# yaomy533/pose_estimation

Measured on AMD Instinct MI355X. Metric: crops/sec at 640×480 RGB-D, 1000 sampled pts; ADD(-S) AUC vs reference, higher is better.
Workload: dtype f32; 1 GPU; LineMOD 'cat' batch=64/GPU, 120x120 crops from 640x480 RGB-D, HRNet-W18 + 1000-pt fusion + TBase, PnP-RANSAC (H=100) on GPU; batch_per_gpu=64, global_batch=64, crop=120, points=1000, backbone=hrnet_w18, parallelism=single, graph=True, micro_batches=1, pipeline=none, graph_branches=True

## Files before the change

pose_estimation_amd/csrc/winograd4.hip:

```cpp
#include "krrn_common.h"
#include "krrn_split.h"

namespace {

constexpr int kGX = 16, kGY = 2, kT = kGX * kGY;
constexpr int kN = 64;
constexpr int kC = 8;
constexpr int kRR = 4 * kGY + 2, kRC = 4 * kGX + 2;
constexpr int kRS = 152;
constexpr int kRing = 1536;
constexpr int kRingF = kRing * 4;
constexpr int kVMH = 36 * 64 * 4;
constexpr int kVL = 36 * 64 * 2;
constexpr int kET = kN * 4;
constexpr unsigned kOOB = 0xFFFF0000u;
constexpr int kRawK = 6;
constexpr int kGap = 6;
static_assert(kRR * kRS <= kRing && kRing == 3 * 512, "raw ring");
static_assert(2 * (kRC - 1) + 1 + (kRC - 1) / 4 < kRS && (kRS * 4) % 16 == 0, "padded raw row");
constexpr int kOffL = 2 * kVMH * 4;
constexpr int kOffR = kOffL + 2 * kVL * 4;
constexpr int kLdsBytes = kOffR + 2 * kRingF * 4;
static_assert(36 * 16 * kET <= kLdsBytes, "epilogue (16 tiles) fits the LDS");

struct Wino4Args {
  const float* in;
  int in_cs, in_co;
  int B, H, W, cin;
  long long img;
  const void* U3;
  int N, n_store;
  const float* scale;
  const float* bias;
  const float* res;
  int res_cs, res_co;
  float* out;
  int out_cs, out_co;
  int relu;
  int vec;
  int Ht, Wt;
  const float* w1;
  float* part;
};

template <int CTRL>
__device__ __forceinline__ float dpp_f(float x) {
  return __int_as_float(__builtin_amdgcn_update_dpp(0, __float_as_int(x), CTRL, 0xF, 0xF, false));
}

__device__ __forceinline__ u32x6 split3(const f32x4 x) {
  const KrrnSplit3 s = krrn_split3(x);
  return u32x6{s.m0, s.m1, s.h0, s.h1, s.l0, s.l1};
}

template <int K, typename V>
__device__ __forceinline__ V bt_row(const V (&x)[6]) {
// ... 1 lines not shown
#pragma unroll
  for (int e = 0; e < (int)(sizeof(V) / 4); ++e) {
    if constexpr (K == 0) y[e] = __builtin_fmaf(4.f, x[0][e], __builtin_fmaf(-5.f, x[2][e], x[4][e]));
    if constexpr (K == 1) y[e] = __builtin_fmaf(-4.f, x[1][e] + x[2][e], x[3][e] + x[4][e]);
    if constexpr (K == 2) y[e] = __builtin_fmaf(4.f, x[1][e] - x[2][e], x[4][e] - x[3][e]);
    if constexpr (K == 3) y[e] = __builtin_fmaf(2.f, x[3][e] - x[1][e], x[4][e] - x[2][e]);
    if constexpr (K == 4) y[e] = __builtin_fmaf(2.f, x[1][e] - x[3][e], x[4][e] - x[2][e]);
    if constexpr (K == 5) y[e] = __builtin_fmaf(4.f, x[1][e], __builtin_fmaf(-5.f, x[3][e], x[5][e]));
  }
  return y;
}
template <int K>
__device__ __forceinline__ constexpr bool bt_uses(int c) {
  return K == 0 ? (c == 0 || c == 2 || c == 4) : (K == 5 ? (c == 1 || c == 3 || c == 5) : (c >= 1 && c <= 4));
}

template <int I>
__device__ __forceinline__ f32x4 at_row(const f32x4 (&x)[6]) {
  f32x4 y;
#pragma unroll
  for (int e = 0; e < 4; ++e) {
    if constexpr (I == 0) y[e] = ((x[0][e] + x[1][e]) + x[2][e]) + (x[3][e] + x[4][e]);
    if constexpr (I == 1) y[e] = __builtin_fmaf(2.f, x[3][e] - x[4][e], x[1][e] - x[2][e]);
    if constexpr (I == 2) y[e] = __builtin_fmaf(4.f, x[3][e] + x[4][e], x[1][e] + x[2][e]);
    if constexpr (I == 3) y[e] = __builtin_fmaf(8.f, x[3][e] - x[4][e], x[1][e] - x[2][e]) + x[5][e];
  }
  return y;
}
template <int I>
__device__ __forceinline__ constexpr bool at_uses(int u) {
  return I == 0 ? (u <= 4) : (I == 3 ? (u >= 1) : (u >= 1 && u <= 4));
}

template <int I, int HP>
__device__ __forceinline__ void epi_row(const Wino4Args& a, const char* E, int nq, int tl, int pass, int b, int ty0,
                                        int tx0, int ng, int nb) {
  const char* eb = E + tl * kET + nq * 16;
  f32x4 t[6];
#pragma unroll
  for (int v = 0; v < 6; ++v) {
    f32x4 m[6];
#pragma unroll
    for (int u = 0; u < 6; ++u)
      m[u] = at_uses<I>(u) ? *reinterpret_cast<const f32x4*>(eb + (6 * u + v) * 16 * kET) : f32x4{0.f, 0.f, 0.f, 0.f};
    t[v] = at_row<I>(m);
    asm volatile("" : "+v"(t[v])::"memory");
  }
  f32x4 y[4];
  y[0] = at_row<0>(t);
  y[1] = at_row<1>(t);
  y[2] = at_row<2>(t);
  y[3] = at_row<3>(t);
  const int tile = 16 * pass + tl;
  const int ty = ty0 + (tile >> 4), tx = tx0 + (tile & 15);
  const int oy = 4 * ty + I;
  const int nj = min(4, a.W - 4 * tx);
  if constexpr (HP > 0) {
    const bool ok = ty < a.Ht && oy < a.H && nj > 0 && ng < a.n_store;
    const f32x4 zero = {0.f, 0.f, 0.f, 0.f};
    const f32x4 scl = ok && a.scale ? *reinterpret_cast<const f32x4*>(a.scale + ng) : f32x4{1.f, 1.f, 1.f, 1.f};
    const f32x4 bia = ok && a.bias ? *reinterpret_cast<const f32x4*>(a.bias + ng) : zero;
    f32x4 w[HP];
#pragma unroll
    for (int o = 0; o < HP; ++o) w[o] = ok ? *reinterpret_cast<const f32x4*>(a.w1 + (size_t)o * a.N + ng) : zero;
    const long long pix = ((long long)b * a.H + oy) * a.W + 4 * tx;
    float s[4][HP];
#pragma unroll
    for (int j = 0; j < 4; ++j) {
      const bool okj = ok && j < nj;
      f32x4 v;
#pragma unroll
      for (int e = 0; e < 4; ++e) v[e] = __builtin_fmaf(y[j][e], scl[e], bia[e]);
      if (a.res && okj) v += *reinterpret_cast<const f32x4*>(a.res + (pix + j) * a.res_cs + a.res_co + ng);
      if (a.relu) {
#pragma unroll
        for (int e = 0; e < 4; ++e) v[e] = fmaxf(v[e], 0.f);
      }
      if (!okj) v = zero;
#pragma unroll
      for (int o = 0; o < HP; ++o) s[j][o] = v[0] * w[o][0] + v[1] * w[o][1] + v[2] * w[o][2] + v[3] * w[o][3];
    }
    const bool b0 = nq & 1, b1 = (nq >> 1) & 1;
    float t1[2][HP];
#pragma unroll
    for (int jj = 0; jj < 2; ++jj)
#pragma unroll
      for (int o = 0; o < HP; ++o) {
// ... 37 lines not shown
      }
      *reinterpret_cast<f32x4*>(o + j * a.out_cs) = v;
    }
    return;
  }
#pragma unroll
  for (int e = 0; e < 4; ++e) {
    if (ng + e >= a.n_store) break;
    const float scl = a.scale ? a.scale[ng + e] : 1.f, bia = a.bias ? a.bias[ng + e] : 0.f;
#pragma unroll
    for (int j = 0; j < 4; ++j) {
      if (j >= nj) break;
      float v = __builtin_fmaf(y[j][e], scl, bia);
      if (rs) v += rs[j * a.res_cs + e];
      if (a.relu) v = fmaxf(v, 0.f);
      o[j * a.out_cs + e] = v;
    }
  }
}

__global__ __launch_bounds__(256) void wino4_head_finish_kernel(const float* __restrict__ part, int nbn, long long M,
                                                                int HW, const float* __restrict__ b1, int p1,
                                                                float* __restrict__ out, int out_c) {
  const long long m = (long long)blockIdx.x * 256 + threadIdx.x;
  if (m >= M) return;
  f32x4 v = *reinterpret_cast<const f32x4*>(part + m * 4);
  for (int nb = 1; nb < nbn; ++nb) v += *reinterpret_cast<const f32x4*>(part + ((size_t)nb * M + m) * 4);
  const long long b = m / HW, p = m - b * HW;
#pragma unroll
  for (int o = 0; o < 4; ++o)
    if (o < p1) out[(b * out_c + o) * HW + p] = v[o] + (b1 ? b1[o] : 0.f);
}

template <int HP>
__global__ __launch_bounds__(512, 1) void wino_f43_x3_kernel(const Wino4Args a) {
  __shared__ __attribute__((aligned(16))) char smem[kLdsBytes];
  const int tid = threadIdx.x, lane = tid & 63;
  const int wave = __builtin_amdgcn_readfirstlane(tid >> 6);
  const int gxn = krrn_cdiv(a.Wt, kGX), gyn = krrn_cdiv(a.Ht, kGY), nbn = krrn_cdiv(a.N, kN);
  const int per_img = gxn * gyn;
  const int bid = krrn_xcd_remap(blockIdx.x, a.B * per_img * nbn);
  const int sp = bid / nbn, nb = bid - (bid / nbn) * nbn;
  const int b = sp / per_img, r2 = sp - (sp / per_img) * per_img;
  const int by = r2 / gxn, bx = r2 - (r2 / gxn) * gxn;
  const int n0 = nb * kN;
  const int ty0 = by * kGY, tx0 = bx * kGX;
  const int nck = a.cin / kC;

  const __amdgpu_buffer_rsrc_t rsA = __builtin_amdgcn_make_buffer_rsrc(
      (void*)(a.in + (size_t)b * a.img + a.in_co), (short)0, (int)min(a.img * 4 - (long long)a.in_co * 4, 0x7FFFFFFFLL),
      0x00020000);
  unsigned roff[3];
#pragma unroll
  for (int i = 0; i < 3; ++i) {
    const int s = 192 * wave + 64 * i + lane;
    const int r = s / kRS, q = s - (s / kRS) * kRS;
    const int g4 = q / 9, w9 = q - (q / 9) * 9;
    const int col = 4 * g4 + (w9 >> 1), hh = w9 & 1;
    const int iy = 4 * ty0 - 1 + r, ix = 4 * tx0 - 1 + col;
    const bool ok = r < kRR && w9 < 8 && col < kRC && iy >= 0 && iy < a.H && ix >= 0 && ix < a.W;
    roff[i] = ok ? (unsigned)((((long long)iy * a.W + ix) * a.in_cs + 4 * hh) * 4) : kOOB;
  }
  auto dma_raw = [&](int ck, int slot) {
    char* dst = smem + kOffR + slot * (kRingF * 4) + 3 * 1024 * wave;
#pragma unroll
    for (int i = 0; i < 3; ++i)
      __builtin_amdgcn_raw_ptr_buffer_load_lds(rsA, (__attribute__((address_space(3))) void*)(dst + 1024 * i), 16,
                                               roff[i], ck * kC * 4, 0, 0);
  };

  const int g = wave & 3, nh = wave >> 2;
  const int cu0 = 3 * (g >> 1), cv0 = 3 * (g & 1);
  const int fr = lane & 31, h = lane >> 5;
  const long long nrec = (long long)nck * 36 * a.N * 2;
  const char* u3 = reinterpret_cast<const char*>(a.U3);
  const __amdgpu_buffer_rsrc_t rsMH =
      __builtin_amdgcn_make_buffer_rsrc((void*)u3, (short)0, (int)min(nrec * 16, 0x7FFFFFFFLL), 0x00020000);
  const __amdgpu_buffer_rsrc_t rsL =
      __builtin_amdgcn_make_buffer_rsrc((void*)(u3 + nrec * 16), (short)0, (int)min(nrec * 8, 0x7FFFFFFFLL), 0x00020000);
  const unsigned wrec = (unsigned)(2 * min(n0 + 32 * nh + fr, a.N - 1) + h);
  u32x4 wmh[3];
  u32x2 wl[3];
  auto load_w = [&](int ck, int k) {
    ck = min(ck, nck - 1);
    const int comp = 6 * (cu0 + k / 3) + cv0 + k % 3;
    const unsigned srec = (unsigned)((ck * 36 + comp) * a.N * 2);
    wmh[k % 3] = __builtin_bit_cast(u32x4, __builtin_amdgcn_raw_buffer_load_b128(rsMH, wrec * 16u, srec * 16u, 0));
    wl[k % 3] = __builtin_bit_cast(u32x2, __builtin_amdgcn_raw_buffer_load_b64(rsL, wrec * 8u, srec * 8u, 0));
  };

  f32x16 acc[9];
#pragma unroll
  for (int k = 0; k < 9; ++k)
#pragma unroll
    for (int r = 0; r < 16; ++r) acc[k][r] = 0.f;

  const int tv = wave < 6 ? wave : 5;
  int tcol[4];
  float tk[4];
  switch (tv) {
    case 0: tcol[0] = 0; tcol[1] = 2; tcol[2] = 4; tcol[3] = 4; tk[0] = 4.f; tk[1] = -5.f; tk[2] = 1.f; tk[3] = 0.f; break;
    case 1: tcol[0] = 1; tcol[1] = 2; tcol[2] = 3; tcol[3] = 4; tk[0] = -4.f; tk[1] = -4.f; tk[2] = 1.f; tk[3] = 1.f; break;
    case 2: tcol[0] = 1; tcol[1] = 2; tcol[2] = 3; tcol[3] = 4; tk[0] = 4.f; tk[1] = -4.f; tk[2] = -1.f; tk[3] = 1.f; break;
    case 3: tcol[0] = 1; tcol[1] = 2; tcol[2] = 3; tcol[3] = 4; tk[0] = -2.f; tk[1] = -1.f; tk[2] = 2.f; tk[3] = 1.f; break;
    case 4: tcol[0] = 1; tcol[1] = 2; tcol[2] = 3; tcol[3] = 4; tk[0] = 2.f; tk[1] = -1.f; tk[2] = -2.f; tk[3] = 1.f; break;
    default: tcol[0] = 1; tcol[1] = 3; tcol[2] = 5; tcol[3] = 5; tk[0] = 4.f; tk[1] = -5.f; tk[2] = 1.f; tk[3] = 0.f; break;
  }
  const int ttile = lane & 31, th = lane >> 5;
  const int pbase = (4 * (ttile >> 4)) * kRS + 9 * (ttile & 15) + th;
  const char* tb[4];
  char* twm = nullptr;
  char* twl = nullptr;
  f32x4 td[4];
  f32x4 te[6];
  auto t_begin = [&](int ck) {
    const int p = ck & 1;
    const char* rb = smem + kOffR + p * (kRingF * 4) + 16 * pbase;
#pragma unroll
    for (int t = 0; t < 4; ++t) tb[t] = rb + 16 * (2 * tcol[t] + (tcol[t] >> 2));
    twm = smem + p * (kVMH * 4) + tv * 1024 + 16 * lane;
    twl = smem + kOffL + p * (kVL * 4) + tv * 512 + 8 * lane;
#pragma unroll
    for (int t = 0; t < 4; ++t) td[t] = *reinterpret_cast<const f32x4*>(tb[t]);
  };
  auto t_step = [&](int s) {
    if (s < 6) {
#pragma unroll
      for (int e = 0; e < 4; ++e)
        te[s][e] = __builtin_fmaf(tk[3], td[3][e], __builtin_fmaf(tk[2], td[2][e], __builtin_fmaf(tk[1], td[1][e], tk[0] * td[0][e])));
      if (s < 5) {
#pragma unroll
        for (int t = 0; t < 4; ++t) {
          (void)tv;
          td[t] = *reinterpret_cast<const f32x4*>(tb[t] + (s + 1) * kRS * 16);
        }
      }
      return;
    }
    const int u = s - 6;
    f32x4 x;
    switch (u) {
      case 0: x = bt_row<0>(te); break;
      case 1: x = bt_row<1>(te); break;
      case 2: x = bt_row<2>(te); break;
      case 3: x = bt_row<3>(te); break;
      case 4: x = bt_row<4>(te); break;
      default: x = bt_row<5>(te); break;
    }
    const u32x6 ch = split3(x);
    *reinterpret_cast<u32x4*>(twm + 6 * u * 1024) = u32x4{ch[0], ch[1], ch[2], ch[3]};
    *reinterpret_cast<u32x2*>(twl + 6 * u * 512) = u32x2{ch[4], ch[5]};
  };
  constexpr int kStep0[10] = {0, 1, 2, 3, 4, 5, 7, 9, 11, 12};

  auto comp_of = [&](int k) { return 6 * (cu0 + k / 3) + cv0 + k % 3; };
  auto do_chunk = [&](int ck) {
    const bool tr = ck + 1 < nck && wave < 6;
    const int p = ck & 1;
    const char* vm = smem + p * (kVMH * 4) + 16 * lane;
    const char* vlo = smem + kOffL + p * (kVL * 4) + 8 * lane;
    auto chain = [&](int k) {
      const u32x4 mh = *reinterpret_cast<const u32x4*>(vm + comp_of(k) * 1024);
      const u32x2 l = *reinterpret_cast<const u32x2*>(vlo + comp_of(k) * 512);
      return u32x6{mh[0], mh[1], mh[2], mh[3], l[0], l[1]};
    };
    const bool stage = ck + 2 < nck;
    __builtin_amdgcn_sched_barrier(0);
    if (tr) t_begin(ck + 1 < nck ? ck + 1 : ck + 1 - 2);
    u32x6 acn = chain(0);
#pragma unroll
    for (int k = 0; k < 9; ++k) {
      u32x6 ac = acn;
      if (k < 8) acn = chain(k + 1);
      asm volatile("" : "+v"(ac));
      u32x6 bc = {wmh[k % 3][0], wmh[k % 3][1], wmh[k % 3][2], wmh[k % 3][3], wl[k % 3][0], wl[k % 3][1]};
      asm volatile("" : "+v"(bc));
      acc[k] = __builtin_amdgcn_mfma_f32_32x32x16_bf16(krrn_sub4(ac, 0), krrn_sub4(bc, 0), acc[k], 0, 0, 0);
      acc[k] = __builtin_amdgcn_mfma_f32_32x32x16_bf16(krrn_sub4(ac, 0), krrn_sub4(bc, 2), acc[k], 0, 0, 0);
      acc[k] = __builtin_amdgcn_mfma_f32_32x32x16_bf16(krrn_sub4(ac, 2), krrn_sub4(bc, 0), acc[k], 0, 0, 0);
      if (k < 6) load_w(ck, k + 3); else load_w(ck + 1, k - 6);
      if (tr) {
#pragma unroll
        for (int st = kStep0[k]; st < kStep0[k + 1]; ++st) t_step(st);
      }
      if (k == kRawK && stage) dma_raw(ck + 2, p);
      __builtin_amdgcn_sched_group_barrier(0x100, 6, 0);
      __builtin_amdgcn_sched_group_barrier(0x008, 1, 0);
      __builtin_amdgcn_sched_group_barrier(0x002, kGap, 0);
      __builtin_amdgcn_sched_group_barrier(0x008, 1, 0);
      __builtin_amdgcn_sched_group_barrier(0x002, kGap, 0);
      __builtin_amdgcn_sched_group_barrier(0x008, 1, 0);
      __builtin_amdgcn_sched_group_barrier(0x002, kGap, 0);
      __builtin_amdgcn_sched_barrier(0);
    }
  };

  dma_raw(0, 0);
  if (nck > 1) dma_raw(1, 1);
#pragma unroll
  for (int k = 0; k < 3; ++k) load_w(0, k);
  if (nck > 1)
    asm volatile("s_waitcnt vmcnt(9)\n\ts_barrier" ::: "memory");
  else
    asm volatile("s_waitcnt vmcnt(6)\n\ts_barrier" ::: "memory");
  if (wave < 6) {
    t_begin(0);
#pragma unroll
    for (int st = 0; st < 12; ++st) t_step(st);
  }
  asm volatile("s_waitcnt vmcnt(6) lgkmcnt(0)\n\ts_barrier" ::: "memory");

  for (int ck = 0; ck < nck; ++ck) {
    do_chunk(ck);
    static_assert(kRawK >= 6 && kRawK <= 8, "vmcnt count below");
    asm volatile("s_waitcnt vmcnt(%0) lgkmcnt(0)\n\ts_barrier" ::"n"(2 * (8 - kRawK)) : "memory");
  }

  const int enq = lane & 15, etl = lane >> 4, ei = wave & 3;
#pragma unroll
  for (int pass = 0; pass < 2; ++pass) {
    char* ew = smem + (32 * nh + fr) * 4;
#pragma unroll
    for (int k = 0; k < 9; ++k) {
      const int comp = comp_of(k);
#pragma unroll
      for (int q = 0; q < 8; ++q) {
        const int r = 8 * pass + q;
        const int tl = (r & 3) + 8 * ((r >> 2) & 1) + 4 * h;
        *reinterpret_cast<float*>(ew + (comp * 16 + tl) * kET) = acc[k][r];
      }
    }
    __syncthreads();
#pragma unroll
    for (int it = 0; it < 2; ++it) {
      const int tl = 4 * ((wave >> 2) + 2 * it) + etl;
      const int ng = n0 + 4 * enq;
      switch (ei) {
        case 0: epi_row<0, HP>(a, smem, enq, tl, pass, b, ty0, tx0, ng, nb); break;
        case 1: epi_row<1, HP>(a, smem, enq, tl, pass, b, ty0, tx0, ng, nb); break;
        case 2: epi_row<2, HP>(a, smem, enq, tl, pass, b, ty0, tx0, ng, nb); break;
        default: epi_row<3, HP>(a, smem, enq, tl, pass, b, ty0, tx0, ng, nb); break;
      }
    }
    __syncthreads();
  }
}

}

KRRN_API int krrn_conv3x3_wino4_x3_f32(const float* in, int in_cs, int in_co, int B, int H, int W, int cin,
                                       const void* U3, int N, int n_store, const float* scale, const float* bias,
                                       const float* res, int res_cs, int res_co, float* out, int out_cs, int out_co,
                                       int relu, void* stream) {
  if (!in || !U3 || !out) return KRRN_EARG;
  if (B < 1 || H < 1 || W < 1 || N < 1 || n_store < 1 || n_store > N) return KRRN_ESHAPE;
  if (cin < kC || (cin % kC) || in_co + cin > in_cs) return KRRN_EALIGN;
  if (!krrn_aligned16(U3) || (((uintptr_t)in) & 15u) || (in_cs & 3) || (in_co & 3)) return KRRN_EALIGN;
  if (out_co + n_store > out_cs) return KRRN_ESHAPE;
  Wino4Args a;
  a.in = in; a.in_cs = in_cs; a.in_co = in_co; a.B = B; a.H = H; a.W = W; a.cin = cin;
  a.img = (long long)H * W * in_cs;
  a.U3 = U3; a.N = N; a.n_store = n_store; a.scale = scale; a.bias = bias;
  a.res = res; a.res_cs = res_cs; a.res_co = res_co;
  a.out = out; a.out_cs = out_cs; a.out_co = out_co; a.relu = relu;
  a.Ht = (H + 3) / 4; a.Wt = (W + 3) / 4;
  const bool ov = !(out_cs & 3) && !(out_co & 3) && krrn_aligned16(out);
  const bool rv = !res || (!(res_cs & 3) && !(res_co & 3) && krrn_aligned16(res));
  const bool sv = (!scale || krrn_aligned16(scale)) && (!bias || krrn_aligned16(bias));
  a.vec = (ov && rv && sv) ? 1 : 0;
  a.w1 = nullptr; a.part = nullptr;
  const long long nrec = (long long)(cin / kC) * 36 * N * 2;
  if (a.img * 4 >= 0x7FFF0000LL || nrec * 16 >= 0x7FFF0000LL) return KRRN_ESHAPE;
  const long long rb = (long long)B * krrn_cdiv(a.Ht, kGY) * krrn_cdiv(a.Wt, kGX) * krrn_cdiv(N, kN);
  if (rb > 0x7fffffffLL) return KRRN_ESHAPE;
  hipLaunchKernelGGL(wino_f43_x3_kernel<0>, dim3((unsigned)rb), dim3(512), 0, (hipStream_t)stream, a);
  return krrn_launch_status();
}

KRRN_API int krrn_conv3x3_wino4_x3_head_f32(const float* in, int in_cs, int in_co, int B, int H, int W, int cin,
                                            const void* U3, int N, const float* scale, const float* bias,
                                            const float* res, int res_cs, int res_co, int relu, const float* w1,
                                            const float* b1, int p1, float* part, float* out, int out_c,
                                            void* stream) {
  if (!in || !U3 || !w1 || !part || !out) return KRRN_EARG;
  if (B < 1 || H < 1 || W < 1 || N < 4 || (N & 3) || p1 < 1 || p1 > 4 || out_c < p1) return KRRN_ESHAPE;
  if (cin < kC || (cin % kC) || in_co + cin > in_cs) return KRRN_EALIGN;
  if (!krrn_aligned16(U3) || (((uintptr_t)in) & 15u) || (in_cs & 3) || (in_co & 3)) return KRRN_EALIGN;
  if (!krrn_aligned16(w1) || !krrn_aligned16(part)) return KRRN_EALIGN;
  if ((scale && !krrn_aligned16(scale)) || (bias && !krrn_aligned16(bias))) return KRRN_EALIGN;
  if (res && ((res_cs & 3) || (res_co & 3) || !krrn_aligned16(res))) return KRRN_EALIGN;
  Wino4Args a;
  a.in = in; a.in_cs = in_cs; a.in_co = in_co; a.B = B; a.H = H; a.W = W; a.cin = cin;
  a.img = (long long)H * W * in_cs;
  a.U3 = U3; a.N = N; a.n_store = N; a.scale = scale; a.bias = bias;
  a.res = res; a.res_cs = res_cs; a.res_co = res_co;
  a.out = nullptr; a.out_cs = 0; a.out_co = 0; a.relu = relu; a.vec = 1;
  a.Ht = (H + 3) / 4; a.Wt = (W + 3) / 4;
  a.w1 = w1; a.part = part;
  const long long nrec = (long long)(cin / kC) * 36 * N * 2;
  if (a.img * 4 >= 0x7FFF0000LL || nrec * 16 >= 0x7FFF0000LL) return KRRN_ESHAPE;
  const int nbn = krrn_cdiv(N, kN);
  const long long rb = (long long)B * krrn_cdiv(a.Ht, kGY) * krrn_cdiv(a.Wt, kGX) * nbn;
  const long long M = (long long)B * H * W;
  const long long fb = (M + 255) / 256;
  if (rb > 0x7fffffffLL || fb > 0x7fffffffLL) return KRRN_ESHAPE;
  hipStream_t s = (hipStream_t)stream;
  if (p1 <= 3) hipLaunchKernelGGL(wino_f43_x3_kernel<3>, dim3((unsigned)rb), dim3(512), 0, s, a);
  else hipLaunchKernelGGL(wino_f43_x3_kernel<4>, dim3((unsigned)rb), dim3(512), 0, s, a);
  const int st = krrn_launch_status();
  if (st != KRRN_OK) return st;
  hipLaunchKernelGGL(wino4_head_finish_kernel, dim3((unsigned)fb), dim3(256), 0, s, part, nbn, M, H * W, b1, p1, out,
                     out_c);
  return krrn_launch_status();
}
```

pose_estimation_amd/hrnet.py:

```python
from __future__ import annotations

from typing import List, Optional, Tuple

import torch
import torch.nn as nn

from . import knobs, ops
from .config import load_hrnet_spec
from .ops import Act, pad4
from .runtime import add_conv_group, add_gemm, Plan, add_conv, ptr

FUSE_EDGES = knobs.flag("KRRN_FUSE_EDGES")
FUSE_EARLY = knobs.flag("KRRN_FUSE_EARLY")
MODULE_STREAMS = knobs.flag("KRRN_MODULE_STREAMS")
STAGE_STREAMS = knobs.flag("KRRN_STAGE_STREAMS")
CONVT_KCHUNK = 16

BN_MOMENTUM = 0.1


def conv3x3(cin, cout, stride=1):
    return nn.Conv2d(cin, cout, kernel_size=3, stride=stride, padding=1, bias=False)


# ... 121 lines not shown
                if cur[i] != pre[i]:
                    layers.append(nn.Sequential(nn.Conv2d(pre[i], cur[i], 3, 1, 1, bias=False),
                                                nn.BatchNorm2d(cur[i]), nn.ReLU(True)))
                else:
                    layers.append(None)
            else:
                chain = []
                for j in range(i + 1 - len(pre)):
                    cin = pre[-1]
                    cout = cur[i] if j == i - len(pre) else cin
                    chain.append(nn.Sequential(nn.Conv2d(cin, cout, 3, 2, 1, bias=False), nn.BatchNorm2d(cout),
                                               nn.ReLU(True)))
                layers.append(nn.Sequential(*chain))
        return nn.ModuleList(layers)


def build_hrnet(cfg) -> HRNet:
    return HRNet(load_hrnet_spec(cfg.Module.BACKBONE), cfg.Module.BACKBONE_OUTC)



class _Builder:
    def __init__(self, plan: Plan, B: int):
        self.plan = plan
        self.B = B
        self.dev = plan.device
        self.specs = []

    def act(self, H, W, c, cs=None) -> Act:
        cs = pad4(c) if cs is None else cs
        t = self.plan.buf((self.B, H, W, cs))
        return Act(t, self.B, H, W, cs, 0, c)

    def conv(self, x: Act, conv: nn.Module, bn: Optional[nn.Module], out: Optional[Act] = None,
             res: Optional[Act] = None, relu: bool = False, cin_map=None) -> Act:
        if isinstance(conv, nn.ConvTranspose2d):
            spec = ops.make_convT(conv, bn, self.dev, cin_map=cin_map, cin_p=x.cp)
        else:
            spec = ops.make_conv(conv, bn, self.dev, cin_map=cin_map, cin_p=x.cp)
        self.specs.append(spec)
        Ho, Wo = ops.conv_out_hw(spec, x.H, x.W)
        if out is None:
            out = self.act(Ho, Wo, spec.cout)
        assert (out.H, out.W) == (Ho, Wo) and out.cp >= pad4(spec.cout)
        wino = ops.wino_eligible(spec, x.B * Ho * Wo)
        if wino and ops.wino4_eligible(spec, x, Ho, Wo):
            self.emit_wino(x, conv, spec, out, res, relu, f4=True, cin_map=cin_map)
        elif wino and x.cs % 2 == 0 and x.co % 2 == 0:
            self.emit_wino(x, conv, spec, out, res, relu, f4=False, cin_map=cin_map)
        elif ops.small_conv_eligible(spec, x):
            self.emit_small(x, spec, out, res, relu)
        elif not self.emit_gemm(x, spec, out, res, relu):
            self.emit_conv(x, spec, out, res, relu)
        return out

    def wino_problem(self, x: Act, conv: nn.Conv2d, spec, f4: bool, cin_map=None) -> Tuple[torch.Tensor, dict]:
        t, comps = (4, 36) if f4 else (2, 16)
        np_ = pad4(spec.cout)
        U = ops.wino_weights_x3((ops.wino4_weights if f4 else ops.wino_weights)(conv, self.dev, cin_map=cin_map,
                                                                                cin_p=x.cp))
        self.specs.append(U)
        pipe = 2.0 * comps * spec.cin_p * np_ * x.B * ((x.H + t - 1) // t) * ((x.W + t - 1) // t)
        return U, dict(kernel="wino_f43_x3" if f4 else "wino_f23_x3", M=x.B * x.H * x.W, N=np_, K=spec.cin_p * 9,
                       mfma_flops=pipe * 6 / 16, mfma_bf16_flops=pipe * 6)

    def conv_head(self, x: Act, conv: nn.Module, bn: Optional[nn.Module], final: nn.Conv2d, out: torch.Tensor,
                  n_store: int) -> bool:
        if not (isinstance(conv, nn.Conv2d) and tuple(final.kernel_size) == (1, 1)
                and tuple(final.stride) == (1, 1) and final.in_channels == conv.out_channels
                and n_store <= min(4, final.out_channels) and x.cs % 2 == 0 and x.co % 2 == 0):
            return False
        spec = ops.make_conv(conv, bn, self.dev, cin_p=x.cp)
        M = x.B * x.H * x.W
        if not ops.wino_eligible(spec, M):
            return False
        np_ = pad4(spec.cout)
        f4 = ops.wino4_eligible(spec, x, x.H, x.W)
        U, meta = self.wino_problem(x, conv, spec, f4)
        w1 = torch.zeros(4, np_, device=self.dev)
        w1[:final.out_channels, :spec.cout] = final.weight.detach().reshape(final.out_channels, -1).float().to(self.dev)
        b1 = None
        if final.bias is not None:
            b1 = torch.zeros(4, device=self.dev)
            b1[:final.out_channels] = final.bias.detach().float().to(self.dev)
        self.specs += [spec, w1] + ([b1] if b1 is not None else [])
        part = self.plan.scratch(((np_ + 63) // 64) * M * 4)
        meta.update(kernel=meta["kernel"] + "_head", tag="conv_wino_head",
                    flops=2.0 * spec.cin * spec.cout * 9 * M + 2.0 * spec.cout * n_store * M)
        self.plan.add("krrn_conv3x3_wino4_x3_head_f32" if f4 else "krrn_conv3x3_wino_x3_head_f32", ptr(x.t), x.cs,
                      x.co, x.B, x.H, x.W, spec.cin_p, ptr(U), np_,
                      ptr(spec.scale), ptr(spec.bias), ptr(None), 0, 0, 1, ptr(w1), ptr(b1), n_store, ptr(part),
                      ptr(out), out.shape[1], meta=meta)
        return True

    def upsample2(self, x: Act) -> Act:
        up = self.act(2 * x.H, 2 * x.W, x.c)
        self.resize(x, up, align=True)
        return up

    def emit_gemm(self, x: Act, spec, out: Act, res: Optional[Act], relu: bool) -> bool:
        if not (spec.kind == "conv" and spec.ksize == 1 and spec.stride == 1 and out.co == 0
                and (res is None or res.co == 0)):
            return False
        np_ = pad4(spec.cout)
        return add_gemm(self.plan, a=x.t, a_off=x.co, lda=x.cs, M=x.B * x.H * x.W, wt=spec.wt[0], K=spec.cin_p,
                        N=np_, scale=spec.scale, bias=spec.bias, out=out.t, ldo=out.cs, relu=relu,
                        res=res.t if res is not None else None, ldr=res.cs if res is not None else 0,
                        cin=spec.cin, cout=spec.cout, tag="conv1x1_gemm")

    @staticmethod
    def small_problem(x: Act, spec, out: Act, res: Optional[Act], relu: bool) -> dict:
        np_ = pad4(spec.cout)
        M = x.B * out.H * out.W
        taps = spec.ksize * spec.ksize
        ntiles = (np_ + 15) // 16
        nw, ks = ops.small_conv_config(M, ntiles, spec.cin_p)
        ksteps = (taps * spec.cin_p // 4 + 3) // 4
        return dict(x=ptr(x.t), in_cs=x.cs, in_co=x.co, B=x.B, H=x.H, W=x.W, cin=spec.cin_p, wt=ptr(spec.wt[0]),
                    N=np_, n_store=np_, scale=ptr(spec.scale), bias=ptr(spec.bias),
                    res=ptr(res.t) if res is not None else ptr(None), res_cs=res.cs if res is not None else 0,
                    res_co=res.co if res is not None else 0, out=ptr(out.t), out_cs=out.cs, out_co=out.co,
                    relu=int(relu), ksize=spec.ksize, stride=spec.stride, nw=nw, ks=ks, M=M,
                    flops=2.0 * spec.cin * spec.cout * taps * M,
                    mfma_flops=2.0 * 16 * ksteps * ops.small_conv_rows(np_, ksteps, ks) * M)

    def emit_small(self, x: Act, spec, out: Act, res: Optional[Act], relu: bool, tag: str = "conv"):
        p = self.small_problem(x, spec, out, res, relu)
        self.plan.add("krrn_conv_small_f32", p["x"], p["in_cs"], p["in_co"], p["B"], p["H"], p["W"], p["cin"], p["wt"],
                      p["N"], p["n_store"], p["scale"], p["bias"], p["res"], p["res_cs"], p["res_co"], p["out"],
                      p["out_cs"], p["out_co"], p["relu"], p["ksize"], p["stride"], p["nw"], p["ks"],
                      meta=dict(kernel=f"conv_small<{p['nw']},{p['ks']}>", flops=p["flops"], tag=tag, M=p["M"], N=p["N"],
                                K=spec.cin_p * spec.ksize ** 2, splits=1, mfma_flops=p["mfma_flops"]))

    def emit_wino(self, x: Act, conv: nn.Conv2d, spec, out: Act, res: Optional[Act], relu: bool, f4: bool,
                  cin_map=None):
        U, meta = self.wino_problem(x, conv, spec, f4, cin_map)
        np_ = meta["N"]
        meta.update(flops=2.0 * spec.cin * spec.cout * 9 * meta["M"], tag="conv_wino")
        self.plan.add("krrn_conv3x3_wino4_x3_f32" if f4 else "krrn_conv3x3_wino_x3_f32", ptr(x.t), x.cs, x.co, x.B,
                      x.H, x.W, spec.cin_p, ptr(U), np_, np_, ptr(spec.scale), ptr(spec.bias),
                      ptr(res.t) if res is not None else ptr(None), res.cs if res is not None else 0,
                      res.co if res is not None else 0, ptr(out.t), out.cs, out.co, int(relu), meta=meta)

    def emit_convT_s2(self, x: Act, spec, out: Act, relu: bool, tag: str = "conv"):
        U3, table = ops.convT_weights_x3(spec)
        self.specs.append(U3)
        taps = sum(len(t) for t in spec.taps)
        grid = x.B * (-(-x.H // 4) * 4) * (-(-x.W // 32) * 32)
        issued = 2.0 * grid * 128 * spec.cin_p * max(len(t) for t in spec.taps) * 4
        meta = dict(kernel="convt_s2_x3", flops=2.0 * spec.cin * spec.cout * taps * x.B * x.H * x.W,
                    tag=tag + "_convT", M=x.B * x.H * x.W * 4, N=128, K=spec.cin_p * taps,
                    mfma_flops=issued * 6 / 16, mfma_bf16_flops=issued * 6)
        self.plan.add("krrn_convT_s2_x3_f32", ptr(x.t), x.cs, x.co, x.B, x.H, x.W, spec.cin_p, table, ptr(U3), 128,
                      ptr(spec.scale), ptr(spec.bias), int(relu), ptr(out.t), out.cs, out.co, out.H, out.W, meta=meta)

    def emit_conv(self, x: Act, spec, out: Act, res: Optional[Act], relu: bool, tag: str = "conv"):
        np_ = pad4(spec.cout)
        if ops.convT_s2_eligible(spec, x, out, res):
            self.emit_convT_s2(x, spec, out, relu, tag)
            return
        if spec.kind == "convT" and 1 < len(spec.taps) <= 4:
            probs = [dict(x=ptr(x.t), x_cs=x.cs, x_co=x.co, B=x.B, Hi=x.H, Wi=x.W, cin_p=spec.cin_p, Hg=x.H, Wg=x.W,
                          in_s=1, taps=taps, wt=ptr(spec.wt[cls]), N=np_, n_store=np_, scale=ptr(spec.scale),
                          bias=ptr(spec.bias), res=ptr(res.t) if res is not None else None,
                          res_cs=res.cs if res is not None else 0, res_co=res.co if res is not None else 0,
                          out=ptr(out.t), out_cs=out.cs, out_co=out.co, Ho=out.H, Wo=out.W, osy=2, osx=2, ooy=ooy,
                          oox=oox, relu=relu, cin=spec.cin, cout=spec.cout)
                     for cls, (taps, (ooy, oox)) in enumerate(zip(spec.taps, spec.cls_off))]
            q = CONVT_KCHUNK if CONVT_KCHUNK and spec.cin_p % CONVT_KCHUNK == 0 else 0
            wts = [ops.kchunk_weights(w, len(t), spec.cin_p, q) for w, t in zip(spec.wt, spec.taps)] if q else spec.wt
            for pr in probs:
                pr["k_chunk"] = q
            for pr, cls in zip(probs, range(len(probs))):
                w3 = ops.conv_weights_x3(wts[cls])
                self.specs.append(w3)
# ... 211 lines not shown
```

pose_estimation_amd/krrn.py:

```python
from __future__ import annotations

import ctypes
from collections import OrderedDict

from typing import Dict, List, Optional, Sequence, Tuple

import torch
import torch.nn as nn

from . import knobs, ops
from .config import CONFIG
from .fusion import FEAT_SID, FusionNetLite, build_fusion_plan, emit_fusion_cloud_part, level_sizes
from .hrnet import _Builder, build_hrnet, build_hrnet_plan
from .ops import Act, pad4
from .posenet import PoseNet, build_tbase_plan, emit_pair_compact, emit_tbase_level1
from .runtime import Late, Plan, RngStream, add_conv, h2d, ptr



TBASE_EARLY = knobs.flag("KRRN_TBASE_EARLY")
GRAPH = knobs.flag("KRRN_GRAPH")
FUSION_EARLY = knobs.flag("KRRN_FUSION_EARLY")


# ... 108 lines not shown
                    tb_pre.update(emit_tbase_level1(model.pose.t_net, plan, B, N, N1, fb["feat1"], fb["feat2"],
                                                      cls_key="cls", inc_r=cfg.Module.POSENet.INC_R, num_cls=C))

            if TBASE_EARLY:
                hooks["level1"].append(tracked(emit_tb_l1))
            tb_pairs = {}
            hooks["pairs"] = [tracked(lambda fb: tb_pairs.update(
                emit_pair_compact(plan, B, N, N1, N2, fb["nn1"], fb["nn2"]) or {}))]
            f0 = len(plan.ops)
            feat, self.fusion_bufs = build_fusion_plan(model.fusion, plan, B, N, self.p9, self.perms, hooks=hooks,
                                                       materialize=model.keep_fusion_feat, early=early)
            self.fusion_op_ids = {id(op) for op in plan.ops[f0:] if id(op) not in side_ids and op.name != "sync"}
            self.fusion_op_ids |= early_ids
            self.feat = feat
            fb = self.fusion_bufs
            levels = dict(fm5=fb["fm5"], feat1=fb["feat1"], feat2=fb["feat2"], nn1=fb["nn1"], nn2=fb["nn2"], N1=N1,
                          N2=N2)
            self.pred_t, self.tbase_bufs = build_tbase_plan(model.pose.t_net, plan, B, N, "cls", "cloud",
                                                            cfg.Module.POSENet.INC_R, C, levels,
                                                            pre=tb_pre or None, pre_sid=tb_sid,
                                                            pairs=tb_pairs or None)
            if feat is not None:
                plan.join([FEAT_SID])
        if pose_hook is not None:
            plan.join([psid])
        self.env = {"cls": self.cls, "cloud": self.cloud}
        self.graph: Optional[torch.cuda.CUDAGraph] = None
        self.warm = False
        self.nbytes = plan_bytes(plan) + plan_bytes(getattr(self, "device_perm_plan", None))

    def _head_tail(self, bld: _Builder, x: Act, convs, final: nn.Conv2d, out: torch.Tensor, n_store: int):
        spec = ops.make_conv(final, None, self.plan.device, cin_p=pad4(convs[-1][0].out_channels))
        bld.specs.append(spec)
        h = bld.upsample2(x)
        for i, (conv, bn) in enumerate(convs):
            if i == len(convs) - 1 and bld.conv_head(h, conv, bn, final, out, n_store):
                return
            h = bld.conv(h, conv, bn, relu=True)
        self._nchw_conv(h, spec, out, n_store)

    def _nchw_conv(self, x: Act, spec, out: torch.Tensor, n_store: int):
        B, Cx, Ho, Wo = out.shape
        np_ = pad4(spec.cout)
        if len(spec.taps[0]) == 1 and spec.stride == 1 and spec.cin_p <= 256 and np_ <= 80:
            name, wt = "krrn_conv1x1_nchw_f32", spec.wt[0]
            if spec.cin_p == 128 and np_ > 48:
                name, wt = "krrn_conv1x1_nchw_x3_f32", ops.quad_weights_x3(spec.wt[0], np_, 128)
                self.plan.buffers.append(wt)
            self.plan.add(name, ptr(x.t), x.cs, x.co, x.B, Ho * Wo, spec.cin_p, ptr(wt), np_,
                          n_store, ptr(spec.scale), ptr(spec.bias), ptr(out), Cx, 0,
                          meta=dict(kernel="conv1x1_nchw", flops=2.0 * spec.cin * n_store * B * Ho * Wo,
                                    tag="head_final", M=B * Ho * Wo, N=np_, K=spec.cin_p, splits=1,
                                    mfma_flops=2.0 * spec.cin_p * 16 * ((np_ + 15) // 16) * B * Ho * Wo))
            return
        add_conv(self.plan, x=ptr(x.t), x_cs=x.cs, x_co=x.co, B=x.B, Hi=x.H, Wi=x.W, cin_p=spec.cin_p, Hg=Ho, Wg=Wo,
                 in_s=spec.stride, taps=spec.taps[0], wt=ptr(spec.wt[0]), N=pad4(spec.cout), n_store=n_store,
                 scale=ptr(spec.scale), bias=ptr(spec.bias), out=ptr(out), out_cs=Cx, out_co=0, Ho=Ho, Wo=Wo,
                 nchw=True, cin=spec.cin, cout=n_store, tag="head_final")

    def load_inputs(self, x, p_emb, choose, cls):
        self.x_in.copy_(x, non_blocking=True)
        if self.opt_pose:
            self.cloud.copy_(p_emb, non_blocking=True)
            self.choose.copy_(choose.reshape(self.B, 1, self.N), non_blocking=True)
        self.cls.copy_(cls.reshape(self.B, 1), non_blocking=True)

    def set_perms(self, perms: Optional[Sequence[torch.Tensor]], mode: str):
        if not self.opt_pose:
            return
        if perms is not None:
            for (k, n, m), p in zip(self.perm_sizes, perms):
# ... 171 lines not shown
```

Baseline: 6766 crops/s.

## Fuse 2x bilinear upsample into Winograd F(4,3) conv input transform for head

Adds an UP variant of the Winograd F(4,3) kernel that reads the half-resolution input directly and folds the bilinear upsample weights into the input transform coefficients. This removes the separate upsample2 kernel and its full-resolution intermediate buffer in the head tail. The tile shape changes to 32x1 with a smaller source window per block, and the transform stage uses precomputed per-tile combined coefficients. In exchange it adds coefficient setup cost and a different LDS window layout, and it relies on the upsample being align-corners bilinear with even output sizes.

```diff
diff --git a/pose_estimation_amd/csrc/winograd4.hip b/pose_estimation_amd/csrc/winograd4.hip
--- a/pose_estimation_amd/csrc/winograd4.hip
+++ b/pose_estimation_amd/csrc/winograd4.hip
@@ -22,6 +22,10 @@
 constexpr int kOffR = kOffL + 2 * kVL * 4;
 constexpr int kLdsBytes = kOffR + 2 * kRingF * 4;
 static_assert(36 * 16 * kET <= kLdsBytes, "epilogue (16 tiles) fits the LDS");
+constexpr int kUGX = 32, kUGY = 1;
+constexpr int kUR = 4, kUC = 66;
+constexpr int kURS = 168;
+static_assert(kUGX * kUGY == kT && 2 * (kUC - 1) + (kUC - 1) / 2 + 1 < kURS && kUR * kURS <= 2 * 512, "source window");
 
 struct Wino4Args {
   const float* in;
@@ -89,7 +93,7 @@
   return I == 0 ? (u <= 4) : (I == 3 ? (u >= 1) : (u >= 1 && u <= 4));
 }
 
-template <int I, int HP>
+template <int I, int HP, bool UP>
 __device__ __forceinline__ void epi_row(const Wino4Args& a, const char* E, int nq, int tl, int pass, int b, int ty0,
                                         int tx0, int ng, int nb) {
   const char* eb = E + tl * kET + nq * 16;
@@ -109,7 +113,7 @@
   y[2] = at_row<2>(t);
   y[3] = at_row<3>(t);
   const int tile = 16 * pass + tl;
-  const int ty = ty0 + (tile >> 4), tx = tx0 + (tile & 15);
+  const int ty = UP ? ty0 : ty0 + (tile >> 4), tx = UP ? tx0 + tile : tx0 + (tile & 15);
   const int oy = 4 * ty + I;
   const int nj = min(4, a.W - 4 * tx);
   if constexpr (HP > 0) {
@@ -213,27 +217,93 @@
     if (o < p1) out[(b * out_c + o) * HW + p] = v[o] + (b1 ? b1[o] : 0.f);
 }
 
-template <int HP>
+__device__ __forceinline__ int up_base(int t, int n_in, float sc) {
+  int i0, i1;
+  float l0, l1;
+  krrn_src_index(max(4 * t - 1, 0), n_in, sc, 1, i0, i1, l0, l1);
+  return i0;
+}
+__device__ __forceinline__ void up_coefs(const float (&bt)[6], int t, int n_in, int n_out, float sc, float (&c)[4]) {
+  const int base = up_base(t, n_in, sc);
+#pragma unroll
+  for (int j = 0; j < 4; ++j) c[j] = 0.f;
+#pragma unroll
+  for (int p = 0; p < 6; ++p) {
+    const int x = 4 * t - 1 + p;
+    int i0, i1;
+    float l0, l1;
+    krrn_src_index(min(max(x, 0), n_out - 1), n_in, sc, 1, i0, i1, l0, l1);
+    const bool in = x >= 0 && x < n_out;
+    const float w0 = in ? bt[p] * l0 : 0.f, w1 = in ? bt[p] * l1 : 0.f;
+#pragma unroll
+    for (int j = 0; j < 4; ++j) c[j] += (i0 - base == j ? w0 : 0.f) + (i1 - base == j ? w1 : 0.f);
+  }
+}
+__device__ __forceinline__ void bt_coefs(int k, float (&b)[6]) {
+  switch (k) {
+    case 0: b[0] = 4.f; b[1] = 0.f; b[2] = -5.f; b[3] = 0.f; b[4] = 1.f; b[5] = 0.f; break;
+    case 1: b[0] = 0.f; b[1] = -4.f; b[2] = -4.f; b[3] = 1.f; b[4] = 1.f; b[5] = 0.f; break;
+    case 2: b[0] = 0.f; b[1] = 4.f; b[2] = -4.f; b[3] = -1.f; b[4] = 1.f; b[5] = 0.f; break;
+    case 3: b[0] = 0.f; b[1] = -2.f; b[2] = -1.f; b[3] = 2.f; b[4] = 1.f; b[5] = 0.f; break;
+    case 4: b[0] = 0.f; b[1] = 2.f; b[2] = -1.f; b[3] = -2.f; b[4] = 1.f; b[5] = 0.f; break;
+    default: b[0] = 0.f; b[1] = 4.f; b[2] = 0.f; b[3] = -5.f; b[4] = 0.f; b[5] = 1.f; break;
+  }
+}
+
+template <int HP, bool UP>
 __global__ __launch_bounds__(512, 1) void wino_f43_x3_kernel(const Wino4Args a) {
   __shared__ __attribute__((aligned(16))) char smem[kLdsBytes];
   const int tid = threadIdx.x, lane = tid & 63;
   const int wave = __builtin_amdgcn_readfirstlane(tid >> 6);
-  const int gxn = krrn_cdiv(a.Wt, kGX), gyn = krrn_cdiv(a.Ht, kGY), nbn = krrn_cdiv(a.N, kN);
+  constexpr int GX = UP ? kUGX : kGX, GY = UP ? kUGY : kGY;
+  const int gxn = krrn_cdiv(a.Wt, GX), gyn = krrn_cdiv(a.Ht, GY), nbn = krrn_cdiv(a.N, kN);
   const int per_img = gxn * gyn;
   const int bid = krrn_xcd_remap(blockIdx.x, a.B * per_img * nbn);
   const int sp = bid / nbn, nb = bid - (bid / nbn) * nbn;
   const int b = sp / per_img, r2 = sp - (sp / per_img) * per_img;
   const int by = r2 / gxn, bx = r2 - (r2 / gxn) * gxn;
   const int n0 = nb * kN;
-  const int ty0 = by * kGY, tx0 = bx * kGX;
+  const int ty0 = by * GY, tx0 = bx * GX;
   const int nck = a.cin / kC;
 
   const __amdgpu_buffer_rsrc_t rsA = __builtin_amdgcn_make_buffer_rsrc(
       (void*)(a.in + (size_t)b * a.img + a.in_co), (short)0, (int)min(a.img * 4 - (long long)a.in_co * 4, 0x7FFFFFFFLL),
       0x00020000);
+  constexpr int ND = UP ? 2 : 3;
+  const int Hi = a.H >> 1, Wi = a.W >> 1;
+  float ucx[4];
+  float ucy[6][4];
+  int urow0 = 0, ucol0 = 0;
+  float usw = 0.f;
+  if constexpr (UP) {
+    const float ush = (float)(Hi - 1) / (float)(a.H - 1);
+    usw = (float)(Wi - 1) / (float)(a.W - 1);
+    urow0 = up_base(ty0, Hi, ush);
+    ucol0 = up_base(tx0, Wi, usw);
+#pragma unroll
+    for (int u = 0; u < 6; ++u) {
+      float bt[6], c[4];
+      bt_coefs(u, bt);
+      up_coefs(bt, ty0, Hi, a.H, ush, c);
+#pragma unroll
+      for (int i = 0; i < 4; ++i) ucy[u][i] = __int_as_float(__builtin_amdgcn_readfirstlane(__float_as_int(c[i])));
+    }
+  }
   unsigned roff[3];
-#pragma unroll
-  for (int i = 0; i < 3; ++i) {
+  if constexpr (UP) {
+#pragma unroll
+    for (int i = 0; i < ND; ++i) {
+      const int s = 64 * ND * wave + 64 * i + lane;
+      const int r = s / kURS, q = s - (s / kURS) * kURS;
+      const int g5 = q / 5, w5 = q - (q / 5) * 5;
+      const int col = 2 * g5 + (w5 >> 1), hh = w5 & 1;
+      const int iy = urow0 + r, ix = ucol0 + col;
+      const bool ok = r < kUR && w5 < 4 && col < kUC && iy < Hi && ix < Wi;
+      roff[i] = ok ? (unsigned)((((long long)iy * Wi + ix) * a.in_cs + 4 * hh) * 4) : kOOB;
+    }
+  }
+#pragma unroll
+  for (int i = 0; i < (UP ? 0 : 3); ++i) {
     const int s = 192 * wave + 64 * i + lane;
     const int r = s / kRS, q = s - (s / kRS) * kRS;
     const int g4 = q / 9, w9 = q - (q / 9) * 9;
@@ -243,9 +313,9 @@
     roff[i] = ok ? (unsigned)((((long long)iy * a.W + ix) * a.in_cs + 4 * hh) * 4) : kOOB;
   }
   auto dma_raw = [&](int ck, int slot) {
-    char* dst = smem + kOffR + slot * (kRingF * 4) + 3 * 1024 * wave;
-#pragma unroll
-    for (int i = 0; i < 3; ++i)
+    char* dst = smem + kOffR + slot * (kRingF * 4) + ND * 1024 * wave;
+#pragma unroll
+    for (int i = 0; i < ND; ++i)
       __builtin_amdgcn_raw_ptr_buffer_load_lds(rsA, (__attribute__((address_space(3))) void*)(dst + 1024 * i), 16,
                                                roff[i], ck * kC * 4, 0, 0);
   };
@@ -288,7 +358,16 @@
     default: tcol[0] = 1; tcol[1] = 3; tcol[2] = 5; tcol[3] = 5; tk[0] = 4.f; tk[1] = -5.f; tk[2] = 1.f; tk[3] = 0.f; break;
   }
   const int ttile = lane & 31, th = lane >> 5;
-  const int pbase = (4 * (ttile >> 4)) * kRS + 9 * (ttile & 15) + th;
+  int pbase = (4 * (ttile >> 4)) * kRS + 9 * (ttile & 15) + th;
+  int podd = 0;
+  if constexpr (UP) {
+    float bt[6];
+    bt_coefs(tv, bt);
+    up_coefs(bt, tx0 + ttile, Wi, a.W, usw, ucx);
+    const int co = min(up_base(tx0 + ttile, Wi, usw) - ucol0, kUC - 4);
+    pbase = 2 * co + (co >> 1) + th;
+    podd = co & 1;
+  }
   const char* tb[4];
   char* twm = nullptr;
   char* twl = nullptr;
@@ -297,14 +376,42 @@
   auto t_begin = [&](int ck) {
     const int p = ck & 1;
     const char* rb = smem + kOffR + p * (kRingF * 4) + 16 * pbase;
-#pragma unroll
-    for (int t = 0; t < 4; ++t) tb[t] = rb + 16 * (2 * tcol[t] + (tcol[t] >> 2));
+    if constexpr (UP) {
+      tb[0] = rb;
+      tb[1] = rb + 16 * (2 + podd);
+      tb[2] = tb[0] + 16 * 5;
+      tb[3] = tb[1] + 16 * 5;
+    } else {
+#pragma unroll
+      for (int t = 0; t < 4; ++t) tb[t] = rb + 16 * (2 * tcol[t] + (tcol[t] >> 2));
+    }
     twm = smem + p * (kVMH * 4) + tv * 1024 + 16 * lane;
     twl = smem + kOffL + p * (kVL * 4) + tv * 512 + 8 * lane;
 #pragma unroll
     for (int t = 0; t < 4; ++t) td[t] = *reinterpret_cast<const f32x4*>(tb[t]);
   };
   auto t_step = [&](int s) {
+    if constexpr (UP) {
+      if (s < 4) {
+#pragma unroll
+        for (int e = 0; e < 4; ++e)
+          te[s][e] = __builtin_fmaf(ucx[3], td[3][e], __builtin_fmaf(ucx[2], td[2][e], __builtin_fmaf(ucx[1], td[1][e], ucx[0] * td[0][e])));
+        if (s < 3) {
+#pragma unroll
+          for (int t = 0; t < 4; ++t) td[t] = *reinterpret_cast<const f32x4*>(tb[t] + (s + 1) * kURS * 16);
+        }
+        return;
+      }
+      const int u = s - 4;
+      f32x4 x;
+#pragma unroll
+      for (int e = 0; e < 4; ++e)
+        x[e] = __builtin_fmaf(ucy[u][3], te[3][e], __builtin_fmaf(ucy[u][2], te[2][e], __builtin_fmaf(ucy[u][1], te[1][e], ucy[u][0] * te[0][e])));
+      const u32x6 ch = split3(x);
+      *reinterpret_cast<u32x4*>(twm + 6 * u * 1024) = u32x4{ch[0], ch[1], ch[2], ch[3]};
+      *reinterpret_cast<u32x2*>(twl + 6 * u * 512) = u32x2{ch[4], ch[5]};
+      return;
+    }
     if (s < 6) {
 #pragma unroll
       for (int e = 0; e < 4; ++e)
@@ -332,7 +439,8 @@
     *reinterpret_cast<u32x4*>(twm + 6 * u * 1024) = u32x4{ch[0], ch[1], ch[2], ch[3]};
     *reinterpret_cast<u32x2*>(twl + 6 * u * 512) = u32x2{ch[4], ch[5]};
   };
-  constexpr int kStep0[10] = {0, 1, 2, 3, 4, 5, 7, 9, 11, 12};
+  constexpr int kStep0[10] = {0, 1, 2, 3, 4, 5, UP ? 6 : 7, UP ? 8 : 9, UP ? 9 : 11, UP ? 10 : 12};
+  constexpr int kSteps = UP ? 10 : 12;
 
   auto comp_of = [&](int k) { return 6 * (cu0 + k / 3) + cv0 + k % 3; };
   auto do_chunk = [&](int ck) {
@@ -381,13 +489,13 @@
 #pragma unroll
   for (int k = 0; k < 3; ++k) load_w(0, k);
   if (nck > 1)
-    asm volatile("s_waitcnt vmcnt(9)\n\ts_barrier" ::: "memory");
+    asm volatile("s_waitcnt vmcnt(%0)\n\ts_barrier" ::"n"(ND + 6) : "memory");
   else
     asm volatile("s_waitcnt vmcnt(6)\n\ts_barrier" ::: "memory");
   if (wave < 6) {
     t_begin(0);
 #pragma unroll
-    for (int st = 0; st < 12; ++st) t_step(st);
+    for (int st = 0; st < kSteps; ++st) t_step(st);
   }
   asm volatile("s_waitcnt vmcnt(6) lgkmcnt(0)\n\ts_barrier" ::: "memory");
 
@@ -417,10 +525,10 @@
       const int tl = 4 * ((wave >> 2) + 2 * it) + etl;
       const int ng = n0 + 4 * enq;
       switch (ei) {
-        case 0: epi_row<0, HP>(a, smem, enq, tl, pass, b, ty0, tx0, ng, nb); break;
-        case 1: epi_row<1, HP>(a, smem, enq, tl, pass, b, ty0, tx0, ng, nb); break;
-        case 2: epi_row<2, HP>(a, smem, enq, tl, pass, b, ty0, tx0, ng, nb); break;
-        default: epi_row<3, HP>(a, smem, enq, tl, pass, b, ty0, tx0, ng, nb); break;
+        case 0: epi_row<0, HP, UP>(a, smem, enq, tl, pass, b, ty0, tx0, ng, nb); break;
+        case 1: epi_row<1, HP, UP>(a, smem, enq, tl, pass, b, ty0, tx0, ng, nb); break;
+        case 2: epi_row<2, HP, UP>(a, smem, enq, tl, pass, b, ty0, tx0, ng, nb); break;
+        default: epi_row<3, HP, UP>(a, smem, enq, tl, pass, b, ty0, tx0, ng, nb); break;
       }
     }
     __syncthreads();
@@ -438,12 +546,14 @@
   if (cin < kC || (cin % kC) || in_co + cin > in_cs) return KRRN_EALIGN;
   if (!krrn_aligned16(U3) || (((uintptr_t)in) & 15u) || (in_cs & 3) || (in_co & 3)) return KRRN_EALIGN;
   if (out_co + n_store > out_cs) return KRRN_ESHAPE;
+  const bool up = relu & 2;
+  if ((relu & ~3) || (up && ((H | W) & 1))) return KRRN_ESHAPE;
   Wino4Args a;
   a.in = in; a.in_cs = in_cs; a.in_co = in_co; a.B = B; a.H = H; a.W = W; a.cin = cin;
-  a.img = (long long)H * W * in_cs;
+  a.img = up ? (long long)(H / 2) * (W / 2) * in_cs : (long long)H * W * in_cs;
   a.U3 = U3; a.N = N; a.n_store = n_store; a.scale = scale; a.bias = bias;
   a.res = res; a.res_cs = res_cs; a.res_co = res_co;
-  a.out = out; a.out_cs = out_cs; a.out_co = out_co; a.relu = relu;
+  a.out = out; a.out_cs = out_cs; a.out_co = out_co; a.relu = relu & 1;
   a.Ht = (H + 3) / 4; a.Wt = (W + 3) / 4;
   const bool ov = !(out_cs & 3) && !(out_co & 3) && krrn_aligned16(out);
   const bool rv = !res || (!(res_cs & 3) && !(res_co & 3) && krrn_aligned16(res));
@@ -452,9 +562,10 @@
   a.w1 = nullptr; a.part = nullptr;
   const long long nrec = (long long)(cin / kC) * 36 * N * 2;
   if (a.img * 4 >= 0x7FFF0000LL || nrec * 16 >= 0x7FFF0000LL) return KRRN_ESHAPE;
-  const long long rb = (long long)B * krrn_cdiv(a.Ht, kGY) * krrn_cdiv(a.Wt, kGX) * krrn_cdiv(N, kN);
+  const long long rb = (long long)B * krrn_cdiv(a.Ht, up ? kUGY : kGY) * krrn_cdiv(a.Wt, up ? kUGX : kGX) * krrn_cdiv(N, kN);
   if (rb > 0x7fffffffLL) return KRRN_ESHAPE;
-  hipLaunchKernelGGL(wino_f43_x3_kernel<0>, dim3((unsigned)rb), dim3(512), 0, (hipStream_t)stream, a);
+  if (up) hipLaunchKernelGGL((wino_f43_x3_kernel<0, true>), dim3((unsigned)rb), dim3(512), 0, (hipStream_t)stream, a);
+  else hipLaunchKernelGGL((wino_f43_x3_kernel<0, false>), dim3((unsigned)rb), dim3(512), 0, (hipStream_t)stream, a);
   return krrn_launch_status();
 }
 
@@ -470,24 +581,28 @@
   if (!krrn_aligned16(w1) || !krrn_aligned16(part)) return KRRN_EALIGN;
   if ((scale && !krrn_aligned16(scale)) || (bias && !krrn_aligned16(bias))) return KRRN_EALIGN;
   if (res && ((res_cs & 3) || (res_co & 3) || !krrn_aligned16(res))) return KRRN_EALIGN;
+  const bool up = relu & 2;
+  if ((relu & ~3) || (up && ((H | W) & 1))) return KRRN_ESHAPE;
   Wino4Args a;
   a.in = in; a.in_cs = in_cs; a.in_co = in_co; a.B = B; a.H = H; a.W = W; a.cin = cin;
-  a.img = (long long)H * W * in_cs;
+  a.img = up ? (long long)(H / 2) * (W / 2) * in_cs : (long long)H * W * in_cs;
   a.U3 = U3; a.N = N; a.n_store = N; a.scale = scale; a.bias = bias;
   a.res = res; a.res_cs = res_cs; a.res_co = res_co;
-  a.out = nullptr; a.out_cs = 0; a.out_co = 0; a.relu = relu; a.vec = 1;
+  a.out = nullptr; a.out_cs = 0; a.out_co = 0; a.relu = relu & 1; a.vec = 1;
   a.Ht = (H + 3) / 4; a.Wt = (W + 3) / 4;
   a.w1 = w1; a.part = part;
   const long long nrec = (long long)(cin / kC) * 36 * N * 2;
   if (a.img * 4 >= 0x7FFF0000LL || nrec * 16 >= 0x7FFF0000LL) return KRRN_ESHAPE;
   const int nbn = krrn_cdiv(N, kN);
-  const long long rb = (long long)B * krrn_cdiv(a.Ht, kGY) * krrn_cdiv(a.Wt, kGX) * nbn;
+  const long long rb = (long long)B * krrn_cdiv(a.Ht, up ? kUGY : kGY) * krrn_cdiv(a.Wt, up ? kUGX : kGX) * nbn;
   const long long M = (long long)B * H * W;
   const long long fb = (M + 255) / 256;
   if (rb > 0x7fffffffLL || fb > 0x7fffffffLL) return KRRN_ESHAPE;
   hipStream_t s = (hipStream_t)stream;
-  if (p1 <= 3) hipLaunchKernelGGL(wino_f43_x3_kernel<3>, dim3((unsigned)rb), dim3(512), 0, s, a);
-  else hipLaunchKernelGGL(wino_f43_x3_kernel<4>, dim3((unsigned)rb), dim3(512), 0, s, a);
+  if (p1 <= 3 && up) hipLaunchKernelGGL((wino_f43_x3_kernel<3, true>), dim3((unsigned)rb), dim3(512), 0, s, a);
+  else if (p1 <= 3) hipLaunchKernelGGL((wino_f43_x3_kernel<3, false>), dim3((unsigned)rb), dim3(512), 0, s, a);
+  else if (up) hipLaunchKernelGGL((wino_f43_x3_kernel<4, true>), dim3((unsigned)rb), dim3(512), 0, s, a);
+  else hipLaunchKernelGGL((wino_f43_x3_kernel<4, false>), dim3((unsigned)rb), dim3(512), 0, s, a);
   const int st = krrn_launch_status();
   if (st != KRRN_OK) return st;
   hipLaunchKernelGGL(wino4_head_finish_kernel, dim3((unsigned)fb), dim3(256), 0, s, part, nbn, M, H * W, b1, p1, out,
diff --git a/pose_estimation_amd/hrnet.py b/pose_estimation_amd/hrnet.py
--- a/pose_estimation_amd/hrnet.py
+++ b/pose_estimation_amd/hrnet.py
@@ -177,20 +177,30 @@
         t = self.plan.buf((self.B, H, W, cs))
         return Act(t, self.B, H, W, cs, 0, c)
 
+    def up2_view(self, x: Act, spec) -> Optional[Act]:
+        v = Act(x.t, x.B, 2 * x.H, 2 * x.W, x.cs, x.co, x.c)
+        if ops.wino_eligible(spec, v.B * v.H * v.W) and ops.wino4_eligible(spec, v, v.H, v.W):
+            return v
+        return None
+
     def conv(self, x: Act, conv: nn.Module, bn: Optional[nn.Module], out: Optional[Act] = None,
-             res: Optional[Act] = None, relu: bool = False, cin_map=None) -> Act:
+             res: Optional[Act] = None, relu: bool = False, cin_map=None, up2: bool = False) -> Act:
         if isinstance(conv, nn.ConvTranspose2d):
             spec = ops.make_convT(conv, bn, self.dev, cin_map=cin_map, cin_p=x.cp)
         else:
             spec = ops.make_conv(conv, bn, self.dev, cin_map=cin_map, cin_p=x.cp)
         self.specs.append(spec)
+        if up2:
+            v = self.up2_view(x, spec)
+            up2 = v is not None
+            x = v if up2 else self.upsample2(x)
         Ho, Wo = ops.conv_out_hw(spec, x.H, x.W)
         if out is None:
             out = self.act(Ho, Wo, spec.cout)
         assert (out.H, out.W) == (Ho, Wo) and out.cp >= pad4(spec.cout)
         wino = ops.wino_eligible(spec, x.B * Ho * Wo)
         if wino and ops.wino4_eligible(spec, x, Ho, Wo):
-            self.emit_wino(x, conv, spec, out, res, relu, f4=True, cin_map=cin_map)
+            self.emit_wino(x, conv, spec, out, res, relu, f4=True, cin_map=cin_map, up2=up2)
         elif wino and x.cs % 2 == 0 and x.co % 2 == 0:
             self.emit_wino(x, conv, spec, out, res, relu, f4=False, cin_map=cin_map)
         elif ops.small_conv_eligible(spec, x):
@@ -210,12 +220,18 @@
                        mfma_flops=pipe * 6 / 16, mfma_bf16_flops=pipe * 6)
 
     def conv_head(self, x: Act, conv: nn.Module, bn: Optional[nn.Module], final: nn.Conv2d, out: torch.Tensor,
-                  n_store: int) -> bool:
+                  n_store: int, up2: bool = False) -> bool:
         if not (isinstance(conv, nn.Conv2d) and tuple(final.kernel_size) == (1, 1)
                 and tuple(final.stride) == (1, 1) and final.in_channels == conv.out_channels
                 and n_store <= min(4, final.out_channels) and x.cs % 2 == 0 and x.co % 2 == 0):
             return False
         spec = ops.make_conv(conv, bn, self.dev, cin_p=x.cp)
+        if up2:
+            if not ops.wino_eligible(spec, 4 * x.B * x.H * x.W):
+                return False
+            v = self.up2_view(x, spec)
+            up2 = v is not None
+            x = v if up2 else self.upsample2(x)
         M = x.B * x.H * x.W
         if not ops.wino_eligible(spec, M):
             return False
@@ -234,7 +250,7 @@
                     flops=2.0 * spec.cin * spec.cout * 9 * M + 2.0 * spec.cout * n_store * M)
         self.plan.add("krrn_conv3x3_wino4_x3_head_f32" if f4 else "krrn_conv3x3_wino_x3_head_f32", ptr(x.t), x.cs,
                       x.co, x.B, x.H, x.W, spec.cin_p, ptr(U), np_,
-                      ptr(spec.scale), ptr(spec.bias), ptr(None), 0, 0, 1, ptr(w1), ptr(b1), n_store, ptr(part),
+                      ptr(spec.scale), ptr(spec.bias), ptr(None), 0, 0, 1 | (2 if up2 else 0), ptr(w1), ptr(b1), n_store, ptr(part),
                       ptr(out), out.shape[1], meta=meta)
         return True
 
@@ -278,14 +294,15 @@
                                 K=spec.cin_p * spec.ksize ** 2, splits=1, mfma_flops=p["mfma_flops"]))
 
     def emit_wino(self, x: Act, conv: nn.Conv2d, spec, out: Act, res: Optional[Act], relu: bool, f4: bool,
-                  cin_map=None):
+                  cin_map=None, up2: bool = False):
+        assert f4 or not up2
         U, meta = self.wino_problem(x, conv, spec, f4, cin_map)
         np_ = meta["N"]
         meta.update(flops=2.0 * spec.cin * spec.cout * 9 * meta["M"], tag="conv_wino")
         self.plan.add("krrn_conv3x3_wino4_x3_f32" if f4 else "krrn_conv3x3_wino_x3_f32", ptr(x.t), x.cs, x.co, x.B,
                       x.H, x.W, spec.cin_p, ptr(U), np_, np_, ptr(spec.scale), ptr(spec.bias),
                       ptr(res.t) if res is not None else ptr(None), res.cs if res is not None else 0,
-                      res.co if res is not None else 0, ptr(out.t), out.cs, out.co, int(relu), meta=meta)
+                      res.co if res is not None else 0, ptr(out.t), out.cs, out.co, int(relu) | (2 if up2 else 0), meta=meta)
 
     def emit_convT_s2(self, x: Act, spec, out: Act, relu: bool, tag: str = "conv"):
         U3, table = ops.convT_weights_x3(spec)
diff --git a/pose_estimation_amd/krrn.py b/pose_estimation_amd/krrn.py
--- a/pose_estimation_amd/krrn.py
+++ b/pose_estimation_amd/krrn.py
@@ -164,11 +164,11 @@
     def _head_tail(self, bld: _Builder, x: Act, convs, final: nn.Conv2d, out: torch.Tensor, n_store: int):
         spec = ops.make_conv(final, None, self.plan.device, cin_p=pad4(convs[-1][0].out_channels))
         bld.specs.append(spec)
-        h = bld.upsample2(x)
+        h = x
         for i, (conv, bn) in enumerate(convs):
-            if i == len(convs) - 1 and bld.conv_head(h, conv, bn, final, out, n_store):
+            if i == len(convs) - 1 and bld.conv_head(h, conv, bn, final, out, n_store, up2=i == 0):
                 return
-            h = bld.conv(h, conv, bn, relu=True)
+            h = bld.conv(h, conv, bn, relu=True, up2=i == 0)
         self._nchw_conv(h, spec, out, n_store)
 
     def _nchw_conv(self, x: Act, spec, out: torch.Tensor, n_store: int):
```

Result: faster. 6999 crops/s, median of 6 (+3.5%).
